# yjh0410/YOLO-Nano

Measured on AMD Instinct MI355X. Metric: images/sec YOLO-Nano-1.0x 416x416 bs=32 inference (network + decode + NMS + host delivery), higher is better.
Workload: dtype f32 (split-f16 MFMA x3, fp32 accumulate); 1 GPU; YOLO-Nano-1.0x 416x416 bs=32/GPU fp32 inference, COCO 80-class head + NMS (BASELINE configs[1]); inputs resident in HBM, kept detections delivered to pinned host memory inside the timed region; global_batch=32, parallelism=image-sharded x1, no collective, rccl_ranks=1, launch_mode=eager, streams_per_gpu=4

## Files before the change

### yolo-nano_amd/csrc/kernels_chain.hip

```cpp
#include "yn_internal.h"
#include "yn_device.h"

#include <cstdlib>
#include <type_traits>

namespace ynk {

template <int WM, int WN, int NT, int V>
__global__ __launch_bounds__(256, 2) void unit_chain_kernel(ChainArgs a)
{
    typedef typename VecT<V>::type vec;
    constexpr int BM = 32 * WM, BN = 32 * NT * WN, KP = 16, BS = BN * 2, B_PER = KP * BN / 512, G = V / 2;
    constexpr int MAXB = (BM * (BN / (2 * G)) + 255) / 256;
    static_assert(WM * WN == 4 && B_PER >= 1, "4 waves");
    extern __shared__ __attribute__((aligned(16))) float uc_smem[];
    const int bf = a.bf, CS = bf + 2, W = a.W, H = a.H, HW = H * W;
    float* T = uc_smem;
    float* Bs = uc_smem + ((BM * CS + 3) & ~3);

    const int t = threadIdx.x, lane = t & 63, wave = t >> 6, l31 = lane & 31, h = lane >> 5;
    const int wm = wave % WM, wn = wave / WM;
    const int m0 = (int)xcd_block(blockIdx.x, gridDim.x) * BM;
    if (m0 >= a.M) return;
    const int nchunks = (bf + 2 * KP - 1) / (2 * KP), kp_total = bf >> 1;

    float4 regA[B_PER], regB[B_PER];
    auto prefetch_b = [&](float4 (&reg)[B_PER], const float* Wp, int c) {
#pragma unroll
        for (int i = 0; i < B_PER; ++i) {
            const int idx = t + 256 * i;
            const int kp = idx / (BN / 2), c4 = idx - kp * (BN / 2);
            const int kpg = c * KP + kp;
            float4 v = make_float4(0.0f, 0.0f, 0.0f, 0.0f);
            if (kpg < kp_total) v = *reinterpret_cast<const float4*>(Wp + ((size_t)kpg * a.Npad + c4 * 2) * 2);
            reg[i] = v;
        }
    };
    auto stage_b = [&](float4 (&reg)[B_PER], int buf) {
#pragma unroll
        for (int i = 0; i < B_PER; ++i) {
            const int idx = t + 256 * i;
            const int kp = idx / (BN / 2), c4 = idx - kp * (BN / 2);
            *reinterpret_cast<float4*>(Bs + buf * KP * BS + kp * BS + c4 * 4) = reg[i];
        }
    };
#ifdef YN_EXP_TIMING
    long long TS[8]; int tsn = 0;
#define YN_TS() TS[tsn++] = __builtin_readcyclecounter()
#else
#define YN_TS()
#endif
    YN_TS();
    float bias2[NT], bias1n[NT];
#pragma unroll
    for (int nt = 0; nt < NT; ++nt) {
        const int n = wn * NT * 32 + nt * 32 + l31;
        bias2[nt] = n < bf ? a.b2[n] : 0.0f;
        bias1n[nt] = (a.Wp1n && n < bf) ? a.b1n[n] : 0.0f;
    }

    const int hipr = bf / (2 * G), jhi = bf >> 1;
    float2 xg[MAXB], xl[MAXB];
    auto x1_prefetch = [&]() {
#pragma unroll
    for (int i = 0; i < MAXB; ++i) {
        const int it = t + 256 * i;
        const int r = it / hipr, j0 = (it - r * hipr) * G;
        const int m = m0 + r < a.M ? m0 + r : a.M - 1;
        xg[i] = make_float2(0.0f, 0.0f); xl[i] = xg[i];
        if (it < BM * hipr) {
            const float* px = a.x1 + (size_t)m * a.x1_ld + a.x1_off + j0;
            if constexpr (G == 2) {
                xg[i] = *reinterpret_cast<const float2*>(px);
                xl[i] = *reinterpret_cast<const float2*>(px + jhi);
            } else {
                xg[i].x = px[0];
                xl[i].x = px[jhi];
            }
        }
    }
    };

    {
        const int cgn = bf / V, ppl = 256 / cgn;
        const int cg = t % cgn, pl = t / cgn, c = cg * V;
        const bool worker = pl < ppl;
        {
            constexpr int R = 4;
            auto issue = [&](int run, vec (&win)[3][R + 2]) {
                const int q0 = m0 + run * R - 1;
#pragma unroll
                for (int dy = 0; dy < 3; ++dy)
#pragma unroll
                    for (int i = 0; i < R + 2; ++i) {
                        int q = q0 + (dy - 1) * W + i;
                        q = q < 0 ? 0 : (q >= a.M ? a.M - 1 : q);
                        win[dy][i] = *reinterpret_cast<const vec*>(a.t1 + (size_t)q * a.t1_ld + a.t1_off + c);
                    }
            };
            vec w[9];
#pragma unroll
            for (int k = 0; k < 9; ++k) w[k] = *reinterpret_cast<const vec*>(a.wdw + k * bf + c);
            const vec bias = *reinterpret_cast<const vec*>(a.bdw + c);
            auto finish = [&](int run, vec (&win)[3][R + 2]) {
                const int mrun = m0 + run * R;
                const int rem0 = (mrun < a.M ? mrun : m0) % HW;
                int y = rem0 / W, x = rem0 - y * W;
#pragma unroll
                for (int i = 0; i < R; ++i) {
                    const int r = run * R + i;
                    const bool live = mrun + i < a.M;
                    const bool yk[3] = {live && y >= 1, live, live && y + 1 < H};
                    const bool xk[3] = {x >= 1, true, x + 1 < W};
                    vec acc = bias;
#pragma unroll
                    for (int ky = 0; ky < 3; ++ky)
#pragma unroll
                        for (int kx = 0; kx < 3; ++kx) {
                            const bool ok = yk[ky] && xk[kx];
                            vec v = win[ky][i + kx];
                            if constexpr (V == 4) v = make_float4(ok ? v.x : 0.0f, ok ? v.y : 0.0f, ok ? v.z : 0.0f, ok ? v.w : 0.0f);
                            else v = make_float2(ok ? v.x : 0.0f, ok ? v.y : 0.0f);
                            vfma(acc, v, w[ky * 3 + kx]);
                        }
                    acc = vact(acc, a.dw_act);
                    float* d = T + r * CS + c;
                    if constexpr (V == 4) {
                        *reinterpret_cast<float2*>(d) = make_float2(acc.x, acc.y);
                        *reinterpret_cast<float2*>(d + 2) = make_float2(acc.z, acc.w);
                    } else {
                        *reinterpret_cast<float2*>(d) = acc;
                    }
                    if (++x == W) { x = 0; if (++y == H) y = 0; }
                }
            };
            vec win[3][R + 2];
            if (worker) issue(pl, win);
            prefetch_b(regA, a.Wp2, 0);
            x1_prefetch();
            stage_b(regA, 0);
            if (nchunks > 1) prefetch_b(regA, a.Wp2, 1);
            if (worker) {
                for (int run = pl; run < BM / R; run += ppl) {
                    finish(run, win);
                    if (run + ppl < BM / R) issue(run + ppl, win);
                }
            }
        }
        for (int r = t; r < BM; r += 256) *reinterpret_cast<float2*>(T + r * CS + bf) = make_float2(0.0f, 0.0f);
    }
    __syncthreads();
    YN_TS();

    f32x16 acc[NT];
// ... 643 lines not shown
        {
            constexpr int pad1 = (AST1 - cin) >> 2;
#pragma unroll
            for (int i0 = 0; i0 < NO * pad1; i0 += 256) {
                const int i = i0 + t;
                if (i0 + 256 > NO * pad1 && i >= NO * pad1) break;
                const int r = i / pad1, c2 = cin + 4 * (i - r * pad1);
                *reinterpret_cast<uint2*>(A3h + r * AST1 + c2) = make_uint2(0u, 0u);
                *reinterpret_cast<uint2*>(A3l + r * AST1 + c2) = make_uint2(0u, 0u);
            }
        }
        {
            float2 yv[NI2][9], acc[NI2];
#pragma unroll
            for (int i = 0; i < NI2; ++i) {
                const int op = dpl + i * ppl, opc = op < NO ? op : 0;
                const int dy = opc / TW, dx = opc - dy * TW;
                const float* yw = T32 + (2 * dy * WW + 2 * dx) * CS + dc;
#pragma unroll
                for (int k = 0; k < 9; ++k) yv[i][k] = *reinterpret_cast<const float2*>(yw + ((k / 3) * WW + k % 3) * CS);
                acc[i] = bd;
            }
#pragma unroll
            for (int k = 0; k < 9; ++k)
#pragma unroll
                for (int i = 0; i < NI2; ++i) vfma(acc[i], yv[i][k], wd[k]);
#pragma unroll
            for (int i = 0; i < NI2; ++i) {
                const int op = dpl + i * ppl;
                if (dworker && op < NO) {
                    if (!RELU) acc[i] = vact(acc[i], a.dw_act);
                    amax = range_track(range_track(amax, acc[i].x), acc[i].y);
                    h16x2 hi, lo;
                    hi[0] = (h16)acc[i].x; hi[1] = (h16)acc[i].y;
                    lo[0] = split_lo(acc[i].x, hi[0]); lo[1] = split_lo(acc[i].y, hi[1]);
                    *reinterpret_cast<h16x2*>(A2h + op * AST2 + dc) = hi;
                    *reinterpret_cast<h16x2*>(A2l + op * AST2 + dc) = lo;
                }
            }
        }
        {
            constexpr int padn = (AST2 - bf) >> 1;
#pragma unroll
            for (int i0 = 0; i0 < NO * padn; i0 += 256) {
                const int i = i0 + t;
                if (i0 + 256 > NO * padn && i >= NO * padn) break;
                const int r = i / padn, c2 = bf + 2 * (i - r * padn);
                *reinterpret_cast<unsigned*>(A2h + r * AST2 + c2) = 0u;
                *reinterpret_cast<unsigned*>(A2l + r * AST2 + c2) = 0u;
            }
        }
        __syncthreads();
        YN_TS();

        f32x16 acc0, acc1;
#pragma unroll
        for (int k = 0; k < 16; ++k) { acc0[k] = 0.0f; acc1[k] = 0.0f; }
        constexpr int PS = 2 * bf;
        if (b1_wave) {
            const h16* Ahb = A3h + l31 * AST1 + h * 8;
            const h16* Alb = A3l + l31 * AST1 + h * 8;
#pragma unroll
            for (int ks = 0; ks < 2; ++ks) {
                const h16x8 ah = *reinterpret_cast<const h16x8*>(Ahb + ks * 16);
                const h16x8 al = *reinterpret_cast<const h16x8*>(Alb + ks * 16);
                split_mfma(ah, al, &g2h[ks], &g2l[ks], acc0, acc1);
            }
        }
        if (pw2_wave) {
            const h16* Ahb = A2h + l31 * AST2 + h * 8;
            const h16* Alb = A2l + l31 * AST2 + h * 8;
#pragma unroll
            for (int ks = 0; ks < KS2; ++ks) {
                const h16x8 ah = *reinterpret_cast<const h16x8*>(Ahb + ks * 16);
                const h16x8 al = *reinterpret_cast<const h16x8*>(Alb + ks * 16);
                split_mfma(ah, al, &g2h[ks], &g2l[ks], acc0, acc1);
            }
        }
        if ((pw2_wave || b1_wave) && nt2 * 32 + l31 < bf) {
            float* prow = PT + (4 * h) * PS + 2 * (nt2 * 32 + l31) + (pw2_wave ? 1 : 0);
            const int act23 = pw2_wave ? a.act2 : a.act3;
#pragma unroll
            for (int r = 0; r < 16; ++r)
                prow[((r & 3) + 8 * (r >> 2)) * PS] = act_pw(split_join(acc0[r], acc1[r]) + bias23, act23);
        }
        __syncthreads();
        if (more) consume();
        {
            char* obase = reinterpret_cast<char*>(a.out);
            const unsigned tile_off = (unsigned)(((b * Ho + oy0) * Wo + ox0) * 2 * bf) * 4u;
            constexpr int PQ = bf / 2, RQ = TW * PQ, NST = (TH * RQ + 255) / 256;
            float4 ov[NST];
#pragma unroll
            for (int i = 0; i < NST; ++i) {
                const int e = t + 256 * i;
                ov[i] = *reinterpret_cast<const float4*>(PT + (e < TH * RQ ? e : 0) * 4);
            }
#pragma unroll
            for (int i = 0; i < NST; ++i) {
                const int e = t + 256 * i;
                const int dy = e / RQ, q = e - dy * RQ, dx = q / PQ;
                if (e < TH * RQ && oy0 + dy < Ho && ox0 + dx < Wo)
                    *reinterpret_cast<float4*>(obase + (tile_off + (unsigned)(dy * Wo * 2 * bf) * 4u + (unsigned)q * 16u)) = ov[i];
            }
        }
        YN_TS();
        if (!more) break;
        tl += GL;
    }
    range_report(a.ovf, amax);
#ifdef YN_EXP_TIMING
    if (t == 0 && (blockIdx.x % 61) == 7 && tsn >= 5)
        printf("downpipe blk %d invariants+window %lld gemm1 %lld dw %lld gemm2+store %lld first tile %lld second %lld\n", (int)blockIdx.x, TS[1] - TS[0], TS[2] - TS[1], TS[3] - TS[2],
               TS[4] - TS[3], TS[4] - TS[0], tsn >= 8 ? TS[7] - TS[4] : -1LL);
#endif
#undef YN_TS
}

static size_t down_unit_pipe_lds(int bf, int cin)
{
    return ((size_t)160 * 40 + (size_t)160 * cin + (size_t)160 * (bf + 2)) * sizeof(float) + 160;
}

bool down_unit_covers(const DownArgs& a)
{
    const bool widths = a.cin == 24 && (a.bf == 58 || a.bf == 24);
    return widths && a.W1h && a.W1l && a.W2h && a.W2l && a.Npad1 == a.Npad2 && a.Npad1 == 32 * ((a.bf + 31) / 32) &&
           !(a.H & 1) && !(a.W & 1) && a.B > 0 && (size_t)a.B * a.H * a.W * (size_t)(a.cin > a.bf / 2 ? a.cin : a.bf / 2) < ((size_t)1 << 30) &&
           a.wdw1 && a.bdw1 && a.W3h && a.W3l && a.b3 && a.Npad3 == a.Npad1;
}

void launch_down_unit(const DownArgs& a, hipStream_t s)
{
    const int Ho = a.H >> 1, Wo = a.W >> 1;
    const unsigned tiles = (unsigned)a.B * ((Ho + 3) / 4) * ((Wo + 7) / 8);
    static unsigned long long attr = 0;
    if (attr_pending(attr)) {
        (void)hipFuncSetAttribute(reinterpret_cast<const void*>(down_unit_pipe_kernel<24, 24, true>), hipFuncAttributeMaxDynamicSharedMemorySize, 160 * 1024);
        (void)hipFuncSetAttribute(reinterpret_cast<const void*>(down_unit_pipe_kernel<24, 58, true>), hipFuncAttributeMaxDynamicSharedMemorySize, 160 * 1024);
        (void)hipFuncSetAttribute(reinterpret_cast<const void*>(down_unit_pipe_kernel<24, 24, false>), hipFuncAttributeMaxDynamicSharedMemorySize, 160 * 1024);
        (void)hipFuncSetAttribute(reinterpret_cast<const void*>(down_unit_pipe_kernel<24, 58, false>), hipFuncAttributeMaxDynamicSharedMemorySize, 160 * 1024);
    }
    constexpr unsigned pipe_g = 1024;
    const size_t plds = down_unit_pipe_lds(a.bf, a.cin);
    unsigned g = xcd_grid(tiles);
    if (g > pipe_g) g = pipe_g;
    const bool relu = a.act1 == 1 && a.act2 == 1 && a.act3 == 1 && a.dw_act == 0 && a.dw1_act == 0;
#define YN_DUP(ci, bw, rl) { set_last_kernel_name("down_unit_pipe_kernel<" #ci "," #bw "," #rl ">"); hipLaunchKernelGGL((down_unit_pipe_kernel<ci, bw, rl>), dim3(g), dim3(256), plds, s, a, (int)tiles); }
    if (a.bf == 24) { if (relu) YN_DUP(24, 24, true) else YN_DUP(24, 24, false) }
    else            { if (relu) YN_DUP(24, 58, true) else YN_DUP(24, 58, false) }
#undef YN_DUP
}

template <int NT, int D>
__global__ __launch_bounds__(256, NT == 1 ? 3 : 1) void down2_kernel(Down2Args a)
{
    constexpr int BM = 32;
    extern __shared__ __attribute__((aligned(16))) float d2_smem[];
    const int bf = a.bf, cin = a.cin;
    const int KQ2 = (bf + 7) >> 3, KQ1 = (cin + 7) >> 3, PS2 = plane_stride(bf), PS1 = plane_stride(cin);
    const int S2 = (KQ2 + 1) >> 1, S1 = (KQ1 + 1) >> 1, S = S2 + S1;
    const bool chain = a.W1nh != nullptr;
    h16* A2h = reinterpret_cast<h16*>(d2_smem);
    h16* A2l = A2h + BM * PS2;
    h16* A1h = A2l + BM * PS2;
    h16* A1l = A1h + BM * PS1;

    const int t = threadIdx.x, lane = t & 63, wave = t >> 6, l31 = lane & 31, h = lane >> 5;
    const int Ho = (a.H - 1) / 2 + 1, Wo = (a.W - 1) / 2 + 1, HWo = Ho * Wo, Mo = a.B * HWo;
    const int m0 = (int)xcd_block(blockIdx.x, gridDim.x) * BM;
    if (m0 >= Mo) return;
    const int nrows = Mo - m0 < BM ? Mo - m0 : BM;

#ifdef YN_EXP_TIMING
    long long TS[8]; int tsn = 0;
#define YN_TS() TS[tsn++] = __builtin_readcyclecounter()
#else
#define YN_TS()
#endif
    YN_TS();
    const int G2 = (S2 + D - 1) / D * D, G1 = (S1 + D - 1) / D * D;
    h16x8 bq[D][NT][2];
    auto load_b = [&](int s, h16x8 (&dst)[NT][2]) {
        const bool second = s >= G2, third = s >= G2 + G1;
        const int ks = third ? s - (G2 + G1) : (second ? s - G2 : s), KQ = (second && !third) ? KQ1 : KQ2;
        const h16* Wh = reinterpret_cast<const h16*>((third && chain) ? a.W1nh : ((second && !third) ? a.W3h : a.W2h));
        const h16* Wl = reinterpret_cast<const h16*>((third && chain) ? a.W1nl : ((second && !third) ? a.W3l : a.W2l));
        const int kq = min(ks * 2 + h, KQ - 1);
#pragma unroll
        for (int nt = 0; nt < NT; ++nt) {
            const int n = min((wave * NT + nt) * 32 + l31, a.Npad - 1);
            const size_t off = ((size_t)kq * a.Npad + n) * 8;
            dst[nt][0] = *reinterpret_cast<const h16x8*>(Wh + off);
            dst[nt][1] = *reinterpret_cast<const h16x8*>(Wl + off);
        }
    };
#pragma unroll
    for (int j = 0; j < D; ++j) load_b(j, bq[j]);
    float amax = 0.0f;
    auto dw_branch = [&](const float* __restrict__ src, int C, const float* __restrict__ wd, const float* __restrict__ bd, int act, h16* Ph, h16* Pl, int PS) {
        const int cqn = C >> 2, ppl = 256 / cqn;
        const int cq = t % cqn, pl = t / cqn, c = cq * 4;
        if (pl < ppl) {
            float4 w[9];
#pragma unroll
            for (int k = 0; k < 9; ++k) w[k] = *reinterpret_cast<const float4*>(wd + k * C + c);
            const float4 bias = *reinterpret_cast<const float4*>(bd + c);
            for (int r0 = pl; r0 < nrows; r0 += 2 * ppl) {
                float4 win[2][9];
#pragma unroll
                for (int u = 0; u < 2; ++u) {
                    const int r = r0 + u * ppl;
                    const int m = m0 + (r < nrows ? r : r0);
                    const int b = m / HWo, rem = m - b * HWo;
                    const int oy = rem / Wo, ox = rem - oy * Wo;
#pragma unroll
                    for (int ky = 0; ky < 3; ++ky) {
                        const int iy = 2 * oy - 1 + ky;
                        const bool yok = iy >= 0 && iy < a.H;
                        const float* rowp = src + ((size_t)(b * a.H + (yok ? iy : 0)) * a.W) * C + c;
#pragma unroll
                        for (int kx = 0; kx < 3; ++kx) {
                            const int ix = 2 * ox - 1 + kx;
                            const bool ok = yok && ix >= 0 && ix < a.W;
                            win[u][ky * 3 + kx] = vmask(*reinterpret_cast<const float4*>(rowp + (size_t)(ok ? ix : 0) * C), opaque_mask(ok));
                        }
                    }
                }
#pragma unroll
                for (int u = 0; u < 2; ++u) {
                    const int r = r0 + u * ppl;
                    if (r < nrows) {
                        float4 acc = bias;
#pragma unroll
                        for (int k = 0; k < 9; ++k) vfma(acc, win[u][k], w[k]);
                        acc = vact(acc, act);
                        const float x4[4] = {acc.x, acc.y, acc.z, acc.w};
                        h16x4 hi, lo;
#pragma unroll
                        for (int j = 0; j < 4; ++j) { amax = range_track(amax, x4[j]); hi[j] = (h16)x4[j]; lo[j] = split_lo(x4[j], hi[j]); }
                        *reinterpret_cast<h16x4*>(Ph + r * PS + c) = hi;
                        *reinterpret_cast<h16x4*>(Pl + r * PS + c) = lo;
                    }
                }
            }
        }
        const int padn = PS - C;
        for (int i = t; i < BM * padn; i += 256) { const int r = i / padn, c2 = C + i - r * padn; Ph[r * PS + c2] = (h16)0.0f; Pl[r * PS + c2] = (h16)0.0f; }
        for (int i = t; i < (BM - nrows) * (C >> 2); i += 256) {
            const int r = nrows + i / (C >> 2), c2 = (i % (C >> 2)) * 4;
            h16x4 z; z[0] = z[1] = z[2] = z[3] = (h16)0.0f;
            *reinterpret_cast<h16x4*>(Ph + r * PS + c2) = z; *reinterpret_cast<h16x4*>(Pl + r * PS + c2) = z;
        }
    };
    dw_branch(a.y1, bf, a.wdw, a.bdw, a.dw_act, A2h, A2l, PS2);
    YN_TS();
    dw_branch(a.x, cin, a.wdw1, a.bdw1, a.dw1_act, A1h, A1l, PS1);
    YN_TS();
    float bias2[NT], bias3[NT], bias1n[NT];
#pragma unroll
    for (int nt = 0; nt < NT; ++nt) {
        const int n = (wave * NT + nt) * 32 + l31;
        bias2[nt] = n < bf ? a.b2[n] : 0.0f;
        bias3[nt] = n < bf ? a.b3[n] : 0.0f;
        bias1n[nt] = (chain && n < bf) ? a.b1n[n] : 0.0f;
    }
    __syncthreads();
    YN_TS();
    range_report(a.ovf, amax);

    f32x16 acc0[NT], acc1[NT];
    float y3[NT][16];
#pragma unroll
    for (int i = 0; i < NT; ++i)
#pragma unroll
        for (int k = 0; k < 16; ++k) { acc0[i][k] = 0.0f; acc1[i][k] = 0.0f; }
    const int jhi = bf >> 1;
    char* out_base = reinterpret_cast<char*>(a.out + (size_t)m0 * (2 * bf));
    auto store_pairs = [&]() {
#pragma unroll
        for (int nt = 0; nt < NT; ++nt) {
            const int n = (wave * NT + nt) * 32 + l31;
            if (n < bf) {
                const bool to_plane = chain && n >= jhi;
#pragma unroll
                for (int r = 0; r < 16; ++r) {
                    const int row = (r & 3) + 8 * (r >> 2) + 4 * h;
                    const float z = apply_act(split_join(acc0[nt][r], acc1[nt][r]) + bias3[nt], a.act3);
                    if (row < nrows) *reinterpret_cast<float2*>(out_base + (unsigned)(row * 2 * bf + 2 * n) * 4u) = make_float2(z, y3[nt][r]);
                    if (to_plane) {
                        const float v0 = z, v1 = y3[nt][r];
                        h16x2 hi, lo;
                        amax = range_track(range_track(amax, v0), v1);
                        hi[0] = (h16)v0; hi[1] = (h16)v1;
                        lo[0] = split_lo(v0, hi[0]); lo[1] = split_lo(v1, hi[1]);
                        *reinterpret_cast<h16x2*>(A2h + row * PS2 + 2 * (n - jhi)) = hi;
                        *reinterpret_cast<h16x2*>(A2l + row * PS2 + 2 * (n - jhi)) = lo;
                    }
                }
            }
        }
    };
    auto run_gemm = [&](const h16* Ah_, const h16* Al_, int PS, int Sn, int p0, int p1) {
        const h16* ahp = Ah_ + l31 * PS + h * 8;
        const h16* alp = Al_ + l31 * PS + h * 8;
        for (int s0 = p0; s0 < p1; s0 += D) {
#pragma unroll
            for (int j = 0; j < D; ++j) {
                const int ks = s0 + j - p0;
                const int a_col = ks < Sn ? ks * 16 : PS - 8 - h * 8;
                const h16x8 ah = *reinterpret_cast<const h16x8*>(ahp + a_col);
                const h16x8 al = *reinterpret_cast<const h16x8*>(alp + a_col);
#pragma unroll
                for (int nt = 0; nt < NT; ++nt) {
                    split_mfma(ah, al, bq[j][nt][0], bq[j][nt][1], acc0[nt], acc1[nt]);
                }
                load_b(s0 + j + D, bq[j]);
            }
        }
    };
    run_gemm(A2h, A2l, PS2, S2, 0, G2);
#pragma unroll
    for (int nt = 0; nt < NT; ++nt)
#pragma unroll
        for (int r = 0; r < 16; ++r) {
            y3[nt][r] = apply_act(split_join(acc0[nt][r], acc1[nt][r]) + bias2[nt], a.act2);
            acc0[nt][r] = 0.0f; acc1[nt][r] = 0.0f;
        }
    run_gemm(A1h, A1l, PS1, S1, G2, G2 + G1);
    if (chain) {
        __syncthreads();
        store_pairs();
        __syncthreads();
        range_report(a.ovf, amax);
#pragma unroll
        for (int nt = 0; nt < NT; ++nt)
#pragma unroll
            for (int r = 0; r < 16; ++r) { acc0[nt][r] = 0.0f; acc1[nt][r] = 0.0f; }
        run_gemm(A2h, A2l, PS2, S2, G2 + G1, G2 + G1 + G2);
    }
    YN_TS();
    if (!chain) {
        store_pairs();
    } else {
#pragma unroll
        for (int nt = 0; nt < NT; ++nt) split_join(acc0[nt], acc1[nt]);
        GemmArgs e{};
        e.out = a.t1n; e.out_ld = bf; e.out_off = 0; e.M = m0 + nrows; e.N = bf; e.Npad = a.Npad; e.bias = a.b1n; e.act = a.act1n; e.pass = nullptr;
        gemm_epilogue<NT>(e, acc0, m0, wave * NT * 32, true, lane, bias1n);
    }
#ifdef YN_EXP_TIMING
    YN_TS();
    if (t == 0 && (blockIdx.x % 97) == 5)
        printf("down2 bf %d blk %d dw2 %lld dw1 %lld sync %lld walk %lld end %lld total %lld\n", bf, (int)blockIdx.x, TS[1] - TS[0], TS[2] - TS[1], TS[3] - TS[2],
               TS[4] - TS[3], TS[5] - TS[4], TS[5] - TS[0]);
#endif
#undef YN_TS
}

static size_t down2_lds(int bf, int cin)
{
    const int PS2 = plane_stride(bf), PS1 = plane_stride(cin);
    return ((size_t)2 * 32 * PS2 + (size_t)2 * 32 * PS1) * 2;
}

bool down2_covers(const Down2Args& a)
{
    return a.x && a.y1 && a.W2h && a.W2l && a.W3h && a.W3l && a.wdw && a.wdw1 && a.bdw && a.bdw1 && a.b2 && a.b3 && a.B > 0 && a.H > 1 && a.W > 1 &&
           a.bf >= 4 && a.cin >= 4 && !(a.bf & 3) && !(a.cin & 3) && a.bf <= 256 && a.cin <= 256 && a.Npad >= a.bf && a.Npad <= 256 &&
           (long)a.B * a.H * a.W * (a.bf > a.cin ? a.bf : a.cin) < (1l << 30);
}

void launch_down2(const Down2Args& a, hipStream_t s)
{
    const int Ho = (a.H - 1) / 2 + 1, Wo = (a.W - 1) / 2 + 1;
    const unsigned tiles = (unsigned)(((long)a.B * Ho * Wo + 31) / 32);
    static unsigned long long attr = 0;
    if (attr_pending(attr)) {
        (void)hipFuncSetAttribute(reinterpret_cast<const void*>(down2_kernel<1, 4>), hipFuncAttributeMaxDynamicSharedMemorySize, 160 * 1024);
        (void)hipFuncSetAttribute(reinterpret_cast<const void*>(down2_kernel<2, 4>), hipFuncAttributeMaxDynamicSharedMemorySize, 160 * 1024);
    }
    if (a.Npad <= 128) { set_last_kernel_name("down2_kernel<1,4>"); hipLaunchKernelGGL((down2_kernel<1, 4>), dim3(xcd_grid(tiles)), dim3(256), down2_lds(a.bf, a.cin), s, a); }
    else               { set_last_kernel_name("down2_kernel<2,4>"); hipLaunchKernelGGL((down2_kernel<2, 4>), dim3(xcd_grid(tiles)), dim3(256), down2_lds(a.bf, a.cin), s, a); }
}

constexpr int DWPW_PLANES = 2 * 32 * 104 * 2;
constexpr int DWPW_WIN = 24 * 1024;
constexpr int DWPW_LDS = DWPW_PLANES + DWPW_WIN;
constexpr unsigned DWPW_SLOTS = 1024;

__device__ __forceinline__ void dwpw_pipe_block(const DwPwArgs& a, unsigned char* smem, unsigned bid, unsigned nblocks)
{
    constexpr int TW = 8, TH = 4, NO = TW * TH, C = 96, KQ = C / 8, KS = KQ / 2, AST = C + 8, R = 4;
    constexpr int WW = TW + 2, WR = TH + 2, CQ = C / 4, NP = 8;
    constexpr unsigned WROW = 4096;
    static_assert(2 * NO * AST * 2 == DWPW_PLANES && WR * WROW == DWPW_WIN && WW * CQ * 16 <= WROW && 3 * NP == 4 * WR, "LDS carve; three wavefronts x two rows");
    typedef float f32x4 __attribute__((ext_vector_type(4)));
    h16* Ah = reinterpret_cast<h16*>(smem);
    h16* Al = Ah + NO * AST;
    const unsigned char* win = smem + DWPW_PLANES;
    const unsigned lds_win = (unsigned)(size_t)(__attribute__((address_space(3))) unsigned char*)smem + (unsigned)DWPW_PLANES;
    const int t = threadIdx.x, lane = t & 63, wave = __builtin_amdgcn_readfirstlane(t >> 6), l31 = lane & 31, h = lane >> 5;
    const int tx_n = (a.W + TW - 1) / TW, ty_n = (a.H + TH - 1) / TH, per_img = tx_n * ty_n;
    const int tiles = a.B * per_img;
    const int TL = (tiles + 7) >> 3, GL = (int)(nblocks >> 3);
    const int tend = ((int)(bid & 7u) + 1) * TL < tiles ? ((int)(bid & 7u) + 1) * TL : tiles;
    const int tile0 = (int)(bid & 7u) * TL + (int)(bid >> 3);
    if (tile0 >= tend) return;

    const int cq = t % CQ, run = t / CQ;
    const int c = cq * 4, ry = run >> 1, rx = (run & 1) * R;
    struct Pos { int b, oy0, ox0; };
    auto decode = [&](int tile) {
        const int b = tile / per_img, trem = tile - b * per_img, ty = trem / tx_n;
        return Pos{__builtin_amdgcn_readfirstlane(b), __builtin_amdgcn_readfirstlane(ty * TH), __builtin_amdgcn_readfirstlane((trem - ty * tx_n) * TW)};
    };
    auto issue = [&](const Pos& p) {
        int tt = t;
        asm volatile("" : "+v"(tt));
        const int ln = tt & 63;
        unsigned xo[4];
#pragma unroll
        for (int k = 0; k < 4; ++k) {
            int q = ln + 64 * k;
            if (k == 3) q = q < WW * CQ - 1 ? q : WW * CQ - 1;
            const int px = q / CQ, qq = q - px * CQ;
            int ix = p.ox0 - 1 + px;
            ix = ix < 0 ? 0 : (ix < a.W ? ix : a.W - 1);
            xo[k] = (unsigned)(ix * C + qq * 4) * 4u;
        }
        const unsigned dst = lds_win + (unsigned)wave * (2u * WROW);
#pragma unroll
        for (int i = 0; i < NP; ++i) {
            int iy = p.oy0 - 1 + 2 * wave + (i >> 2);
            iy = iy < 0 ? 0 : (iy < a.H ? iy : a.H - 1);
            const unsigned row = (unsigned)((p.b * a.H + iy) * a.W) * (unsigned)(C * 4);
            dma16(reinterpret_cast<const char*>(a.in) + row, xo[i & 3], dst + (unsigned)(i >> 2) * WROW + (unsigned)(i & 3) * 1024u);
        }
    };
    int t1 = tile0 + GL < tend ? tile0 + GL : -1;
    Pos cur = decode(tile0), nxt = cur;
    issue(cur);

    f32x4 wd[9];
#pragma unroll
    for (int k = 0; k < 9; ++k) wd[k] = *reinterpret_cast<const f32x4*>(a.wdw + k * C + c);
    f32x4 bd = *reinterpret_cast<const f32x4*>(a.bdw + c);
    h16x8 gh[KS], gl[KS];
#pragma unroll
    for (int ks = 0; ks < KS; ++ks) {
        const size_t off = ((size_t)(ks * 2 + h) * a.Npad + wave * 32 + l31) * 8;
        gh[ks] = *reinterpret_cast<const h16x8*>(reinterpret_cast<const h16*>(a.Wh) + off);
        gl[ks] = *reinterpret_cast<const h16x8*>(reinterpret_cast<const h16*>(a.Wl) + off);
    }
    float gbias = a.bias[wave * 32 + l31];
    static_assert(KS == 6, "23 asm operands");
    asm volatile("s_waitcnt vmcnt(0)"
                 : "+v"(wd[0]), "+v"(wd[1]), "+v"(wd[2]), "+v"(wd[3]), "+v"(wd[4]), "+v"(wd[5]), "+v"(wd[6]), "+v"(wd[7]), "+v"(wd[8]), "+v"(bd), "+v"(gbias),
                   "+v"(gh[0]), "+v"(gh[1]), "+v"(gh[2]), "+v"(gh[3]), "+v"(gh[4]), "+v"(gh[5]), "+v"(gl[0]), "+v"(gl[1]), "+v"(gl[2]), "+v"(gl[3]), "+v"(gl[4]), "+v"(gl[5])
                 :: "memory");
    float amax = 0.0f;
    const int j4 = lane & 3;
    const int nq = wave * 32 + (l31 & ~3);
    const unsigned wbase = (unsigned)ry * WROW + (unsigned)((rx * CQ + cq) * 16);
    auto depthwise = [&](auto masked) {
        constexpr bool MASKED = decltype(masked)::value;
        unsigned wok = 0;
        if constexpr (MASKED) {
            int tt = t;
            asm volatile("" : "+v"(tt));
            const int rn = tt / CQ, oy = cur.oy0 + (rn >> 1), ox = cur.ox0 + (rn & 1) * R;
            const int jlo = ox < 1 ? 1 - ox : 0, jhi = min(max(a.W + 1 - ox, 0), R + 2);
            const int klo = oy < 1 ? 1 - oy : 0, khi = oy < a.H ? min(a.H + 1 - oy, 3) : 0;
            const unsigned xb = jhi > jlo ? (1u << jhi) - (1u << jlo) : 0u, yb = khi > klo ? (1u << khi) - (1u << klo) : 0u;
            wok = ((yb & 1u) ? xb : 0u) | ((yb & 2u) ? xb << (R + 2) : 0u) | ((yb & 4u) ? xb << (2 * (R + 2)) : 0u);
        }
        const unsigned char* wp = win + wbase;
        float4 acc[R];
#pragma unroll
        for (int o = 0; o < R; ++o) acc[o] = make_float4(bd.x, bd.y, bd.z, bd.w);
#pragma unroll
        for (int ky = 0; ky < 3; ++ky) {
            float4 row[R + 2];
#pragma unroll
            for (int j = 0; j < R + 2; ++j) {
                row[j] = *reinterpret_cast<const float4*>(wp + ky * WROW + j * (CQ * 16));
                if constexpr (MASKED) row[j] = vmask(row[j], 0u - ((wok >> (ky * (R + 2) + j)) & 1u));
            }
#pragma unroll
            for (int o = 0; o < R; ++o)
#pragma unroll
                for (int kx = 0; kx < 3; ++kx) {
                    const f32x4 w = wd[ky * 3 + kx];
                    vfma(acc[o], row[o + kx], make_float4(w.x, w.y, w.z, w.w));
                }
        }
#pragma unroll
        for (int o = 0; o < R; ++o) {
            const float4 v = vact(acc[o], a.dw_act);
            const int op = ry * TW + rx + o;
            const float x4[4] = {v.x, v.y, v.z, v.w};
            h16x4 hi, lo;
#pragma unroll
            for (int j = 0; j < 4; ++j) { amax = range_track(amax, x4[j]); hi[j] = (h16)x4[j]; lo[j] = split_lo(x4[j], hi[j]); }
            *reinterpret_cast<h16x4*>(Ah + op * AST + c) = hi;
            *reinterpret_cast<h16x4*>(Al + op * AST + c) = lo;
        }
    };
    lds_barrier();

    for (;;) {
        if (cur.oy0 >= 1 && cur.oy0 + TH < a.H && cur.ox0 >= 1 && cur.ox0 + TW < a.W) depthwise(std::false_type{});
        else depthwise(std::true_type{});
        lds_barrier();
        if (t1 >= 0) { nxt = decode(t1); issue(nxt); }

        f32x16 acc0, acc1;
#pragma unroll
        for (int k = 0; k < 16; ++k) { acc0[k] = 0.0f; acc1[k] = 0.0f; }
        const h16* Ahb = Ah + l31 * AST + h * 8;
        const h16* Alb = Al + l31 * AST + h * 8;
#pragma unroll
        for (int ks = 0; ks < KS; ++ks) {
            const h16x8 ah = *reinterpret_cast<const h16x8*>(Ahb + ks * 16);
            const h16x8 al = *reinterpret_cast<const h16x8*>(Alb + ks * 16);
            split_mfma(ah, al, gh[ks], gl[ks], acc0, acc1);
        }
        char* obase = reinterpret_cast<char*>(a.out);
        const unsigned lane_off = (unsigned)(((cur.b * a.H + cur.oy0) * a.W + cur.ox0 + 4 * h + j4) * C + nq) * 4u;
        const bool xin = cur.ox0 + 4 * h + j4 < a.W;
        float4 ov[4];
#pragma unroll
        for (int g = 0; g < 4; ++g) {
            float v0 = apply_act(split_join(acc0[4 * g + 0], acc1[4 * g + 0]) + gbias, a.act);
// ... 87 lines not shown
```

Baseline: 50090 images/s.

## Specialize down2 kernel for fixed channel counts with pipelined depthwise loads

Adds compile-time specializations of the stride-2 down unit kernel for 116 and 232 channels. With channel counts fixed, the depthwise window loads are software-pipelined across pixels, pixel coordinates come from float-reciprocal division, boundary masks are packed into bits, weight fragment offsets come from a precomputed tile layout, and weight prefetch is deferred or unrolled with scheduling barriers. The goal is to cut index arithmetic and hide global-load latency in the depthwise phase. In exchange it adds more template instances, raises register pressure, and relies on the float division being exact for maps smaller than the guarded size.

```diff
diff --git a/yolo-nano_amd/csrc/kernels_chain.hip b/yolo-nano_amd/csrc/kernels_chain.hip
--- a/yolo-nano_amd/csrc/kernels_chain.hip
+++ b/yolo-nano_amd/csrc/kernels_chain.hip
@@ -1,5 +1,6 @@
 #include "yn_internal.h"
 #include "yn_device.h"
+#include "yn_unit_tile.h"
 
 #include <cstdlib>
 #include <type_traits>
@@ -949,21 +950,22 @@
 #undef YN_DUP
 }
 
-template <int NT, int D>
+template <int NT, int D, int CIN = 0, int BF = 0, bool CHAIN = false>
 __global__ __launch_bounds__(256, NT == 1 ? 3 : 1) void down2_kernel(Down2Args a)
 {
     constexpr int BM = 32;
+    constexpr bool CT = BF > 0;
     extern __shared__ __attribute__((aligned(16))) float d2_smem[];
-    const int bf = a.bf, cin = a.cin;
+    const int bf = CT ? BF : a.bf, cin = CT ? CIN : a.cin;
     const int KQ2 = (bf + 7) >> 3, KQ1 = (cin + 7) >> 3, PS2 = plane_stride(bf), PS1 = plane_stride(cin);
     const int S2 = (KQ2 + 1) >> 1, S1 = (KQ1 + 1) >> 1, S = S2 + S1;
-    const bool chain = a.W1nh != nullptr;
+    const bool chain = CT ? CHAIN : a.W1nh != nullptr;
     h16* A2h = reinterpret_cast<h16*>(d2_smem);
     h16* A2l = A2h + BM * PS2;
     h16* A1h = A2l + BM * PS2;
     h16* A1l = A1h + BM * PS1;
 
-    const int t = threadIdx.x, lane = t & 63, wave = t >> 6, l31 = lane & 31, h = lane >> 5;
+    const int t = threadIdx.x, lane = t & 63, wave = CT ? __builtin_amdgcn_readfirstlane(t >> 6) : t >> 6, l31 = lane & 31, h = lane >> 5;
     const int Ho = (a.H - 1) / 2 + 1, Wo = (a.W - 1) / 2 + 1, HWo = Ho * Wo, Mo = a.B * HWo;
     const int m0 = (int)xcd_block(blockIdx.x, gridDim.x) * BM;
     if (m0 >= Mo) return;
@@ -977,82 +979,210 @@
 #endif
     YN_TS();
     const int G2 = (S2 + D - 1) / D * D, G1 = (S1 + D - 1) / D * D;
+    constexpr unsigned NPAD = 32u * ((BF + 31) / 32);
+    static_assert(!CT || (!(BF & 3) && !(CIN & 3) && BF <= 256 && CIN <= 256 && NPAD == 128u * NT), "down2_covers, and four wavefronts x NT column tiles = Npad");
+    static_assert(!CT || ((((BF + 7) >> 3) + 1) / 2 > D && (((CIN + 7) >> 3) + 1) / 2 > D), "a padded step's slot holds the fragments of a real step");
     h16x8 bq[D][NT][2];
+    unsigned lw = ((unsigned)h * NPAD + (unsigned)(wave * NT * 32 + l31)) * 16u;
+    if constexpr (CT) asm volatile("" : "+v"(lw));
     auto load_b = [&](int s, h16x8 (&dst)[NT][2]) {
-        const bool second = s >= G2, third = s >= G2 + G1;
-        const int ks = third ? s - (G2 + G1) : (second ? s - G2 : s), KQ = (second && !third) ? KQ1 : KQ2;
-        const h16* Wh = reinterpret_cast<const h16*>((third && chain) ? a.W1nh : ((second && !third) ? a.W3h : a.W2h));
-        const h16* Wl = reinterpret_cast<const h16*>((third && chain) ? a.W1nl : ((second && !third) ? a.W3l : a.W2l));
-        const int kq = min(ks * 2 + h, KQ - 1);
-#pragma unroll
-        for (int nt = 0; nt < NT; ++nt) {
-            const int n = min((wave * NT + nt) * 32 + l31, a.Npad - 1);
-            const size_t off = ((size_t)kq * a.Npad + n) * 8;
-            dst[nt][0] = *reinterpret_cast<const h16x8*>(Wh + off);
-            dst[nt][1] = *reinterpret_cast<const h16x8*>(Wl + off);
-        }
-    };
-#pragma unroll
-    for (int j = 0; j < D; ++j) load_b(j, bq[j]);
+        if constexpr (CT) {
+            const int g = s >= G2 + G1 ? 2 : (s >= G2 ? 1 : 0);
+            const int ks = s - (g == 2 ? G2 + G1 : (g == 1 ? G2 : 0));
+            if (s >= G2 + G1 + (CHAIN ? G2 : 0) || ks >= (g == 1 ? S1 : S2)) return;
+            const char* Wh = reinterpret_cast<const char*>(g == 2 ? a.W1nh : (g == 1 ? a.W3h : a.W2h));
+            const char* Wl = reinterpret_cast<const char*>(g == 2 ? a.W1nl : (g == 1 ? a.W3l : a.W2l));
+            const unsigned off = g == 1 ? frag_step_off<((CIN + 7) >> 3), NPAD>(lw, ks, h) : frag_step_off<((BF + 7) >> 3), NPAD>(lw, ks, h);
+#pragma unroll
+            for (int nt = 0; nt < NT; ++nt) {
+                dst[nt][0] = *reinterpret_cast<const h16x8*>(Wh + (off + (unsigned)nt * 512u));
+                dst[nt][1] = *reinterpret_cast<const h16x8*>(Wl + (off + (unsigned)nt * 512u));
+            }
+        } else {
+            const bool second = s >= G2, third = s >= G2 + G1;
+            const int ks = third ? s - (G2 + G1) : (second ? s - G2 : s), KQ = (second && !third) ? KQ1 : KQ2;
+            const h16* Wh = reinterpret_cast<const h16*>((third && chain) ? a.W1nh : ((second && !third) ? a.W3h : a.W2h));
+            const h16* Wl = reinterpret_cast<const h16*>((third && chain) ? a.W1nl : ((second && !third) ? a.W3l : a.W2l));
+            const int kq = min(ks * 2 + h, KQ - 1);
+#pragma unroll
+            for (int nt = 0; nt < NT; ++nt) {
+                const int n = min((wave * NT + nt) * 32 + l31, a.Npad - 1);
+                const size_t off = ((size_t)kq * a.Npad + n) * 8;
+                dst[nt][0] = *reinterpret_cast<const h16x8*>(Wh + off);
+                dst[nt][1] = *reinterpret_cast<const h16x8*>(Wl + off);
+            }
+        }
+    };
+    constexpr bool BQ_FIRST = !CT || NT > 1;
+    if constexpr (BQ_FIRST) {
+#pragma unroll
+        for (int j = 0; j < D; ++j) load_b(j, bq[j]);
+    }
     float amax = 0.0f;
-    auto dw_branch = [&](const float* __restrict__ src, int C, const float* __restrict__ wd, const float* __restrict__ bd, int act, h16* Ph, h16* Pl, int PS) {
-        const int cqn = C >> 2, ppl = 256 / cqn;
-        const int cq = t % cqn, pl = t / cqn, c = cq * 4;
-        if (pl < ppl) {
-            float4 w[9];
-#pragma unroll
-            for (int k = 0; k < 9; ++k) w[k] = *reinterpret_cast<const float4*>(wd + k * C + c);
-            const float4 bias = *reinterpret_cast<const float4*>(bd + c);
-            for (int r0 = pl; r0 < nrows; r0 += 2 * ppl) {
-                float4 win[2][9];
-#pragma unroll
-                for (int u = 0; u < 2; ++u) {
-                    const int r = r0 + u * ppl;
-                    const int m = m0 + (r < nrows ? r : r0);
-                    const int b = m / HWo, rem = m - b * HWo;
-                    const int oy = rem / Wo, ox = rem - oy * Wo;
-#pragma unroll
-                    for (int ky = 0; ky < 3; ++ky) {
-                        const int iy = 2 * oy - 1 + ky;
-                        const bool yok = iy >= 0 && iy < a.H;
-                        const float* rowp = src + ((size_t)(b * a.H + (yok ? iy : 0)) * a.W) * C + c;
-#pragma unroll
-                        for (int kx = 0; kx < 3; ++kx) {
-                            const int ix = 2 * ox - 1 + kx;
-                            const bool ok = yok && ix >= 0 && ix < a.W;
-                            win[u][ky * 3 + kx] = vmask(*reinterpret_cast<const float4*>(rowp + (size_t)(ok ? ix : 0) * C), opaque_mask(ok));
+    auto split_quad = [&](float4 acc, h16* ph, h16* pl, bool st) {
+        float x4[4] = {acc.x, acc.y, acc.z, acc.w};
+        h16x4 hi, lo;
+#pragma unroll
+        for (int j = 0; j < 4; ++j) {
+            if constexpr (CT) asm volatile("" : "+v"(x4[j]));
+            amax = range_track(amax, x4[j]); hi[j] = (h16)x4[j]; lo[j] = split_lo(x4[j], hi[j]);
+        }
+        if (st) {
+            *reinterpret_cast<h16x4*>(ph) = hi;
+            *reinterpret_cast<h16x4*>(pl) = lo;
+        }
+    };
+    if constexpr (CT) {
+        constexpr int CQ2 = BF >> 2, PPL2 = 256 / CQ2, PPT2 = BM / PPL2;
+        constexpr int CQ1 = CIN >> 2, PPL1 = 256 / CQ1, PPT1 = BM / PPL1;
+        constexpr int AH = NT == 1 ? 1 : 2, RT = PPT2 + PPT1;
+        constexpr int CPS2 = plane_stride(BF), CPS1 = plane_stride(CIN);
+        static_assert(BM % PPL2 == 0 && BM % PPL1 == 0, "every pixel lane takes the same number of pixels");
+        const int b0 = m0 / HWo, rem0 = m0 - b0 * HWo;
+        const int y0 = rem0 / Wo, x0 = rem0 - y0 * Wo;
+        const float inv_w = 1.0f / (float)Wo, inv_h = 1.0f / (float)Ho;
+        int t1 = t;
+        asm volatile("" : "+v"(t1));
+        const int cq2 = t % CQ2, pl2_ = t / CQ2, cq1 = t1 % CQ1, pl1_ = t1 / CQ1;
+        const bool on2 = pl2_ < PPL2, on1 = pl1_ < PPL1;
+        const int pl2 = on2 ? pl2_ : 0, pl1 = on1 ? pl1_ : 0, c2 = cq2 * 4, c1 = cq1 * 4;
+        float4 win[AH + 1][9];
+        int okb[AH + 1];
+        auto request = [&](int i) {
+            const bool br1 = i >= PPT2;
+            const int C = br1 ? CIN : BF, r = br1 ? pl1 + (i - PPT2) * PPL1 : pl2 + i * PPL2, c = br1 ? c1 : c2;
+            const char* src = reinterpret_cast<const char*>(br1 ? a.x : a.y1);
+            const int q = x0 + (r < nrows ? r : nrows - 1);
+            const int dy = (int)(((float)q + 0.5f) * inv_w);
+            const int ox = q - dy * Wo, yy = y0 + dy;
+            const int db = (int)(((float)yy + 0.5f) * inv_h);
+            const int oy = yy - db * Ho, b = b0 + db;
+            const int iy = 2 * oy - 1, ix = 2 * ox - 1;
+            const int yb = (iy >= 0 ? 1 : 0) | 2 | (iy + 2 < a.H ? 4 : 0), xb = (ix >= 0 ? 1 : 0) | 2 | (ix + 2 < a.W ? 4 : 0);
+            okb[i % (AH + 1)] = xb * ((yb & 1) + (yb & 2) * 4 + (yb & 4) * 16);
+#pragma unroll
+            for (int ky = 0; ky < 3; ++ky) {
+                const unsigned rowo = (unsigned)((b * a.H + (((yb >> ky) & 1) ? iy + ky : 0)) * a.W);
+#pragma unroll
+                for (int kx = 0; kx < 3; ++kx) {
+                    const bool ok = ((yb >> ky) & 1) && ((xb >> kx) & 1);
+                    const unsigned off = ((rowo + (unsigned)(ok ? ix + kx : 0)) * (unsigned)C + (unsigned)c) * 4u;
+                    win[i % (AH + 1)][ky * 3 + kx] = *reinterpret_cast<const float4*>(src + off);
+                }
+            }
+        };
+        float4 w[9], bias;
+        auto taps = [&](bool br1) {
+            const float* wd = br1 ? a.wdw1 : a.wdw;
+#pragma unroll
+            for (int k = 0; k < 9; ++k) w[k] = *reinterpret_cast<const float4*>(wd + k * (br1 ? CIN : BF) + (br1 ? c1 : c2));
+            bias = *reinterpret_cast<const float4*>((br1 ? a.bdw1 : a.bdw) + (br1 ? c1 : c2));
+        };
+        auto sum = [&](int i) {
+            const bool br1 = i >= PPT2;
+            const int r = br1 ? pl1 + (i - PPT2) * PPL1 : pl2 + i * PPL2;
+            float4 acc = bias;
+#pragma unroll
+            for (int k = 0; k < 9; ++k)
+                vfma(acc, k == 4 ? win[i % (AH + 1)][k] : vmask(win[i % (AH + 1)][k], (unsigned)__builtin_amdgcn_sbfe(okb[i % (AH + 1)], k, 1)), w[k]);
+            acc = vact(acc, br1 ? a.dw1_act : a.dw_act);
+            if (br1) split_quad(acc, A1h + r * CPS1 + c1, A1l + r * CPS1 + c1, on1 && r < nrows);
+            else     split_quad(acc, A2h + r * CPS2 + c2, A2l + r * CPS2 + c2, on2 && r < nrows);
+        };
+#pragma unroll
+        for (int i = 0; i < AH; ++i) request(i);
+        taps(false);
+#pragma unroll
+        for (int i = 0; i < RT; ++i) {
+            if (i + AH < RT) request(i + AH);
+            if (i == PPT2) { YN_TS(); taps(true); }
+            if constexpr (!BQ_FIRST) {
+                if (i == RT - 1) {
+#pragma unroll
+                    for (int j = 0; j < D; ++j) load_b(j, bq[j]);
+                }
+            }
+            __builtin_amdgcn_sched_barrier(0);
+            sum(i);
+            __builtin_amdgcn_sched_barrier(0);
+        }
+        const uint2 z = make_uint2(0u, 0u);
+        constexpr int PQ2 = (CPS2 - BF) >> 2, PQ1 = (CPS1 - CIN) >> 2;
+#pragma unroll
+        for (int i0 = 0; i0 < BM * PQ2; i0 += 256) {
+            const int i = i0 + t, r = i / PQ2, cz = BF + 4 * (i - r * PQ2);
+            if (i < BM * PQ2) { *reinterpret_cast<uint2*>(A2h + r * CPS2 + cz) = z; *reinterpret_cast<uint2*>(A2l + r * CPS2 + cz) = z; }
+        }
+#pragma unroll
+        for (int i0 = 0; i0 < BM * PQ1; i0 += 256) {
+            const int i = i0 + t, r = i / PQ1, cz = CIN + 4 * (i - r * PQ1);
+            if (i < BM * PQ1) { *reinterpret_cast<uint2*>(A1h + r * CPS1 + cz) = z; *reinterpret_cast<uint2*>(A1l + r * CPS1 + cz) = z; }
+        }
+        if (nrows < BM) {
+            for (int i = t; i < (BM - nrows) * CQ2; i += 256) {
+                const int r = nrows + i / CQ2, cz = (i % CQ2) * 4;
+                *reinterpret_cast<uint2*>(A2h + r * CPS2 + cz) = z; *reinterpret_cast<uint2*>(A2l + r * CPS2 + cz) = z;
+            }
+            for (int i = t; i < (BM - nrows) * CQ1; i += 256) {
+                const int r = nrows + i / CQ1, cz = (i % CQ1) * 4;
+                *reinterpret_cast<uint2*>(A1h + r * CPS1 + cz) = z; *reinterpret_cast<uint2*>(A1l + r * CPS1 + cz) = z;
+            }
+        }
+    } else {
+        auto dw_branch = [&](const float* __restrict__ src, int C, const float* __restrict__ wd, const float* __restrict__ bd, int act, h16* Ph, h16* Pl, int PS) {
+            const int cqn = C >> 2, ppl = 256 / cqn;
+            const int cq = t % cqn, pl = t / cqn, c = cq * 4;
+            if (pl < ppl) {
+                float4 w[9];
+#pragma unroll
+                for (int k = 0; k < 9; ++k) w[k] = *reinterpret_cast<const float4*>(wd + k * C + c);
+                const float4 bias = *reinterpret_cast<const float4*>(bd + c);
+                for (int r0 = pl; r0 < nrows; r0 += 2 * ppl) {
+                    float4 win[2][9];
+#pragma unroll
+                    for (int u = 0; u < 2; ++u) {
+                        const int r = r0 + u * ppl;
+                        const int m = m0 + (r < nrows ? r : r0);
+                        const int b = m / HWo, rem = m - b * HWo;
+                        const int oy = rem / Wo, ox = rem - oy * Wo;
+#pragma unroll
+                        for (int ky = 0; ky < 3; ++ky) {
+                            const int iy = 2 * oy - 1 + ky;
+                            const bool yok = iy >= 0 && iy < a.H;
+                            const float* rowp = src + ((size_t)(b * a.H + (yok ? iy : 0)) * a.W) * C + c;
+#pragma unroll
+                            for (int kx = 0; kx < 3; ++kx) {
+                                const int ix = 2 * ox - 1 + kx;
+                                const bool ok = yok && ix >= 0 && ix < a.W;
+                                win[u][ky * 3 + kx] = vmask(*reinterpret_cast<const float4*>(rowp + (size_t)(ok ? ix : 0) * C), opaque_mask(ok));
+                            }
                         }
                     }
-                }
-#pragma unroll
-                for (int u = 0; u < 2; ++u) {
-                    const int r = r0 + u * ppl;
-                    if (r < nrows) {
-                        float4 acc = bias;
-#pragma unroll
-                        for (int k = 0; k < 9; ++k) vfma(acc, win[u][k], w[k]);
-                        acc = vact(acc, act);
-                        const float x4[4] = {acc.x, acc.y, acc.z, acc.w};
-                        h16x4 hi, lo;
-#pragma unroll
-                        for (int j = 0; j < 4; ++j) { amax = range_track(amax, x4[j]); hi[j] = (h16)x4[j]; lo[j] = split_lo(x4[j], hi[j]); }
-                        *reinterpret_cast<h16x4*>(Ph + r * PS + c) = hi;
-                        *reinterpret_cast<h16x4*>(Pl + r * PS + c) = lo;
+#pragma unroll
+                    for (int u = 0; u < 2; ++u) {
+                        const int r = r0 + u * ppl;
+                        if (r < nrows) {
+                            float4 acc = bias;
+#pragma unroll
+                            for (int k = 0; k < 9; ++k) vfma(acc, win[u][k], w[k]);
+                            acc = vact(acc, act);
+                            split_quad(acc, Ph + r * PS + c, Pl + r * PS + c, true);
+                        }
                     }
                 }
             }
-        }
-        const int padn = PS - C;
-        for (int i = t; i < BM * padn; i += 256) { const int r = i / padn, c2 = C + i - r * padn; Ph[r * PS + c2] = (h16)0.0f; Pl[r * PS + c2] = (h16)0.0f; }
-        for (int i = t; i < (BM - nrows) * (C >> 2); i += 256) {
-            const int r = nrows + i / (C >> 2), c2 = (i % (C >> 2)) * 4;
-            h16x4 z; z[0] = z[1] = z[2] = z[3] = (h16)0.0f;
-            *reinterpret_cast<h16x4*>(Ph + r * PS + c2) = z; *reinterpret_cast<h16x4*>(Pl + r * PS + c2) = z;
-        }
-    };
-    dw_branch(a.y1, bf, a.wdw, a.bdw, a.dw_act, A2h, A2l, PS2);
-    YN_TS();
-    dw_branch(a.x, cin, a.wdw1, a.bdw1, a.dw1_act, A1h, A1l, PS1);
+            const int padn = PS - C;
+            for (int i = t; i < BM * padn; i += 256) { const int r = i / padn, c2 = C + i - r * padn; Ph[r * PS + c2] = (h16)0.0f; Pl[r * PS + c2] = (h16)0.0f; }
+            for (int i = t; i < (BM - nrows) * (C >> 2); i += 256) {
+                const int r = nrows + i / (C >> 2), c2 = (i % (C >> 2)) * 4;
+                h16x4 z; z[0] = z[1] = z[2] = z[3] = (h16)0.0f;
+                *reinterpret_cast<h16x4*>(Ph + r * PS + c2) = z; *reinterpret_cast<h16x4*>(Pl + r * PS + c2) = z;
+            }
+        };
+        dw_branch(a.y1, bf, a.wdw, a.bdw, a.dw_act, A2h, A2l, PS2);
+        YN_TS();
+        dw_branch(a.x, cin, a.wdw1, a.bdw1, a.dw1_act, A1h, A1l, PS1);
+    }
     YN_TS();
     float bias2[NT], bias3[NT], bias1n[NT];
 #pragma unroll
@@ -1101,7 +1231,7 @@
     auto run_gemm = [&](const h16* Ah_, const h16* Al_, int PS, int Sn, int p0, int p1) {
         const h16* ahp = Ah_ + l31 * PS + h * 8;
         const h16* alp = Al_ + l31 * PS + h * 8;
-        for (int s0 = p0; s0 < p1; s0 += D) {
+        auto group = [&](int s0) {
 #pragma unroll
             for (int j = 0; j < D; ++j) {
                 const int ks = s0 + j - p0;
@@ -1114,6 +1244,12 @@
                 }
                 load_b(s0 + j + D, bq[j]);
             }
+        };
+        if constexpr (CT) {
+#pragma unroll
+            for (int s0 = p0; s0 < p1; s0 += D) { group(s0); __builtin_amdgcn_sched_barrier(0); }
+        } else {
+            for (int s0 = p0; s0 < p1; s0 += D) group(s0);
         }
     };
     run_gemm(A2h, A2l, PS2, S2, 0, G2);
@@ -1143,7 +1279,7 @@
 #pragma unroll
         for (int nt = 0; nt < NT; ++nt) split_join(acc0[nt], acc1[nt]);
         GemmArgs e{};
-        e.out = a.t1n; e.out_ld = bf; e.out_off = 0; e.M = m0 + nrows; e.N = bf; e.Npad = a.Npad; e.bias = a.b1n; e.act = a.act1n; e.pass = nullptr;
+        e.out = a.t1n; e.out_ld = bf; e.out_off = 0; e.M = m0 + nrows; e.N = bf; e.Npad = CT ? (int)NPAD : a.Npad; e.bias = a.b1n; e.act = a.act1n; e.pass = nullptr;
         gemm_epilogue<NT>(e, acc0, m0, wave * NT * 32, true, lane, bias1n);
     }
 #ifdef YN_EXP_TIMING
@@ -1176,7 +1312,16 @@
     if (attr_pending(attr)) {
         (void)hipFuncSetAttribute(reinterpret_cast<const void*>(down2_kernel<1, 4>), hipFuncAttributeMaxDynamicSharedMemorySize, 160 * 1024);
         (void)hipFuncSetAttribute(reinterpret_cast<const void*>(down2_kernel<2, 4>), hipFuncAttributeMaxDynamicSharedMemorySize, 160 * 1024);
-    }
+        (void)hipFuncSetAttribute(reinterpret_cast<const void*>(down2_kernel<1, 4, 116, 116, false>), hipFuncAttributeMaxDynamicSharedMemorySize, 160 * 1024);
+        (void)hipFuncSetAttribute(reinterpret_cast<const void*>(down2_kernel<1, 4, 116, 116, true>), hipFuncAttributeMaxDynamicSharedMemorySize, 160 * 1024);
+        (void)hipFuncSetAttribute(reinterpret_cast<const void*>(down2_kernel<2, 4, 232, 232, false>), hipFuncAttributeMaxDynamicSharedMemorySize, 160 * 1024);
+        (void)hipFuncSetAttribute(reinterpret_cast<const void*>(down2_kernel<2, 4, 232, 232, true>), hipFuncAttributeMaxDynamicSharedMemorySize, 160 * 1024);
+    }
+    const bool chained = a.W1nh != nullptr, small_map = a.H < 32768 && a.W < 32768;
+#define YN_D2(ci, bw, nt, ch) { set_last_kernel_name("down2_kernel<" #nt ",4>"); hipLaunchKernelGGL((down2_kernel<nt, 4, ci, bw, ch>), dim3(xcd_grid(tiles)), dim3(256), down2_lds(a.bf, a.cin), s, a); return; }
+    if (small_map && a.cin == 116 && a.bf == 116 && a.Npad == 128) { if (chained) YN_D2(116, 116, 1, true) else YN_D2(116, 116, 1, false) }
+    if (small_map && a.cin == 232 && a.bf == 232 && a.Npad == 256) { if (chained) YN_D2(232, 232, 2, true) else YN_D2(232, 232, 2, false) }
+#undef YN_D2
     if (a.Npad <= 128) { set_last_kernel_name("down2_kernel<1,4>"); hipLaunchKernelGGL((down2_kernel<1, 4>), dim3(xcd_grid(tiles)), dim3(256), down2_lds(a.bf, a.cin), s, a); }
     else               { set_last_kernel_name("down2_kernel<2,4>"); hipLaunchKernelGGL((down2_kernel<2, 4>), dim3(xcd_grid(tiles)), dim3(256), down2_lds(a.bf, a.cin), s, a); }
 }
```

New measurement: 50310 images/s, median of 6. Within noise of the previous version (+0.4%).
